# CityU-AIM-Group/SimT

Hardware: AMD Instinct MI355X
Metric: training images/sec at 768x768, DeepLabv2-R101+SimT (higher is better)
Workload: dtype bf16; 1 GPU; DeepLabv2-ResNet101 + SimT(C=19,K=3) full training iteration, batch=4/GPU, 768x768, bf16, 1xMI355X; global_batch=4, inputs=resident in HBM (see h2d_inclusive of a --full run for the PCIe-inclusive rate)

## Files before the change

### simt_amd/csrc/head_expand.hip

```cpp
#include "common.h"

struct TapArgs {
  const void* src;
  const float* bias;
  void* dst;
  int B, H, W, Q, QP, lds, ldd, ntaps;
  long M;
  short dy[SIMT_MAX_TAPS], dx[SIMT_MAX_TAPS];
};

__global__ __launch_bounds__(256) void tap_gather_sum_kernel(TapArgs a) {
  const int nq = a.QP >> 2;
  const long total = a.M * nq;
  const float* P = (const float*)a.src;
  float* y = (float*)a.dst;
  for (long idx = (long)blockIdx.x * blockDim.x + threadIdx.x; idx < total; idx += (long)gridDim.x * blockDim.x) {
    const int q = (int)(idx % nq);
    const long m = idx / nq;
    const int ox = (int)(m % a.W);
    const long t2 = m / a.W;
    const int oy = (int)(t2 % a.H);
    float4 acc = make_float4(0.f, 0.f, 0.f, 0.f);
    if (a.bias) {
      const int c = q * 4;
      acc.x = c + 0 < a.Q ? a.bias[c + 0] : 0.f;
      acc.y = c + 1 < a.Q ? a.bias[c + 1] : 0.f;
      acc.z = c + 2 < a.Q ? a.bias[c + 2] : 0.f;
      acc.w = c + 3 < a.Q ? a.bias[c + 3] : 0.f;
    }
    for (int t = 0; t < a.ntaps; ++t) {
      const int iy = oy + a.dy[t], ix = ox + a.dx[t];
      if (iy < 0 || iy >= a.H || ix < 0 || ix >= a.W) continue;
      const float4 v = *(const float4*)(P + (m + (long)a.dy[t] * a.W + a.dx[t]) * a.lds + t * a.QP + q * 4);
      acc.x += v.x; acc.y += v.y; acc.z += v.z; acc.w += v.w;
    }
    *(float4*)(y + m * a.ldd + q * 4) = acc;
  }
}

__global__ __launch_bounds__(256) void tap_scatter_kernel(TapArgs a) {
  const int ng = a.QP >> 3;
  const long total = a.M * a.ntaps * ng;
  const bf16_t* d = (const bf16_t*)a.src;
  bf16_t* G = (bf16_t*)a.dst;
  for (long idx = (long)blockIdx.x * blockDim.x + threadIdx.x; idx < total; idx += (long)gridDim.x * blockDim.x) {
    const int g = (int)(idx % ng);
    long r = idx / ng;
    const int t = (int)(r % a.ntaps);
    const long m = r / a.ntaps;
    const int ox = (int)(m % a.W);
    const int oy = (int)((m / a.W) % a.H);
    const int iy = oy - a.dy[t], ix = ox - a.dx[t];
    uint4 v = make_uint4(0u, 0u, 0u, 0u);
    if (iy >= 0 && iy < a.H && ix >= 0 && ix < a.W)
      v = *(const uint4*)(d + (m - ((long)a.dy[t] * a.W + a.dx[t])) * a.lds + g * 8);
    st_out16(G + m * a.ldd + t * a.QP + g * 8, v);
  }
}

static int tap_grid(long total) {
  long g = (total + 255) / 256;
  if (g > 256 * 16) g = 256 * 16;
  return (int)(g < 1 ? 1 : g);
}

extern "C" int simt_tap_gather_sum(const simt_tap_desc* d, simt_stream_t stream) {
  SIMT_CHECK(d && d->src && d->dst && d->ntaps >= 1 && d->ntaps <= SIMT_MAX_TAPS);
  SIMT_CHECK(d->QP % 4 == 0 && d->lds % 4 == 0 && d->ldd % 4 == 0 && d->QP <= d->ldd && d->ntaps * d->QP <= d->lds);
  TapArgs a;
  a.src = d->src; a.bias = d->bias; a.dst = d->dst; a.B = d->B; a.H = d->H; a.W = d->W; a.Q = d->Q; a.QP = d->QP;
  a.lds = d->lds; a.ldd = d->ldd; a.ntaps = d->ntaps; a.M = (long)d->B * d->H * d->W;
  for (int i = 0; i < SIMT_MAX_TAPS; ++i) { a.dy[i] = d->dy[i]; a.dx[i] = d->dx[i]; }
  hipLaunchKernelGGL(tap_gather_sum_kernel, dim3(tap_grid(a.M * (a.QP / 4))), dim3(256), 0, (hipStream_t)stream, a);
  SIMT_LAUNCH_CHECK();
  return SIMT_OK;
}

extern "C" int simt_tap_scatter(const simt_tap_desc* d, simt_stream_t stream) {
  SIMT_CHECK(d && d->src && d->dst && d->ntaps >= 1 && d->ntaps <= SIMT_MAX_TAPS);
  SIMT_CHECK(d->QP % 8 == 0 && d->lds % 8 == 0 && d->ldd % 8 == 0 && d->QP <= d->lds && d->ntaps * d->QP <= d->ldd);
  TapArgs a;
  a.src = d->src; a.bias = nullptr; a.dst = d->dst; a.B = d->B; a.H = d->H; a.W = d->W; a.Q = d->Q; a.QP = d->QP;
  a.lds = d->lds; a.ldd = d->ldd; a.ntaps = d->ntaps; a.M = (long)d->B * d->H * d->W;
  for (int i = 0; i < SIMT_MAX_TAPS; ++i) { a.dy[i] = d->dy[i]; a.dx[i] = d->dx[i]; }
  hipLaunchKernelGGL(tap_scatter_kernel, dim3(tap_grid(a.M * a.ntaps * (a.QP / 8))), dim3(256), 0, (hipStream_t)stream, a);
  SIMT_LAUNCH_CHECK();
  return SIMT_OK;
}
```

Before: 175.0 images/s.

## Add unrolled tap gather and row-batched tap scatter kernels with fast divmod

```diff
diff --git a/simt_amd/csrc/head_expand.hip b/simt_amd/csrc/head_expand.hip
--- a/simt_amd/csrc/head_expand.hip
+++ b/simt_amd/csrc/head_expand.hip
@@ -1,3 +1,4 @@
+#define SIMT_NT_STORES 1
 #include "common.h"
 
 struct TapArgs {
@@ -38,6 +39,40 @@
   }
 }
 
+template <int NT>
+__global__ __launch_bounds__(256) void tap_gather_sum_nt_kernel(TapArgs a, int nq, int total, float rcp_nq, float rcp_w, float rcp_h) {
+  const int idx = xcd_remap((int)blockIdx.x, (int)gridDim.x) * 256 + (int)threadIdx.x;
+  if (idx >= total) return;
+  int m, q, t2, ox, b, oy;
+  fast_divmod(idx, nq, rcp_nq, m, q);
+  fast_divmod(m, a.W, rcp_w, t2, ox);
+  fast_divmod(t2, a.H, rcp_h, b, oy);
+  const float* P = (const float*)a.src;
+  const float* own = P + (long)m * a.lds + q * 4;
+  const float* dummy = P + q * 4;
+  float4 v[NT];
+  bool in[NT];
+#pragma unroll
+  for (int t = 0; t < NT; ++t) {
+    const int iy = oy + a.dy[t], ix = ox + a.dx[t];
+    in[t] = iy >= 0 && iy < a.H && ix >= 0 && ix < a.W;
+    const long off = ((long)a.dy[t] * a.W + a.dx[t]) * a.lds + t * a.QP;
+    v[t] = *(const float4*)(in[t] ? own + off : dummy);
+  }
+  float4 acc = make_float4(0.f, 0.f, 0.f, 0.f);
+  if (a.bias) {
+    const int c = q * 4;
+    acc.x = c + 0 < a.Q ? a.bias[c + 0] : 0.f;
+    acc.y = c + 1 < a.Q ? a.bias[c + 1] : 0.f;
+    acc.z = c + 2 < a.Q ? a.bias[c + 2] : 0.f;
+    acc.w = c + 3 < a.Q ? a.bias[c + 3] : 0.f;
+  }
+#pragma unroll
+  for (int t = 0; t < NT; ++t)
+    if (in[t]) { acc.x += v[t].x; acc.y += v[t].y; acc.z += v[t].z; acc.w += v[t].w; }
+  *(float4*)((float*)a.dst + (long)m * a.ldd + q * 4) = acc;
+}
+
 __global__ __launch_bounds__(256) void tap_scatter_kernel(TapArgs a) {
   const int ng = a.QP >> 3;
   const long total = a.M * a.ntaps * ng;
@@ -58,6 +93,39 @@
   }
 }
 
+#ifndef TAP_ROWS
+#define TAP_ROWS 4
+#endif
+__global__ __launch_bounds__(256) void tap_scatter_rows_kernel(TapArgs a, int ng, int np, float rcp_ng, float rcp_w, float rcp_h) {
+  const int lane = (int)threadIdx.x & 63;
+  const int m0 = (xcd_remap((int)blockIdx.x, (int)gridDim.x) * 4 + ((int)threadIdx.x >> 6)) * TAP_ROWS;
+  const int M = (int)a.M;
+  if (m0 >= M) return;
+  int t2, ox0, b, oy0;
+  fast_divmod(m0, a.W, rcp_w, t2, ox0);
+  fast_divmod(t2, a.H, rcp_h, b, oy0);
+  const bf16_t* d = (const bf16_t*)a.src;
+  bf16_t* G = (bf16_t*)a.dst;
+  for (int j = lane; j < np; j += 64) {
+    int t, g;
+    fast_divmod(j, ng, rcp_ng, t, g);
+    const int dyt = a.dy[t], dxt = a.dx[t];
+    const long so = ((long)m0 - ((long)dyt * a.W + dxt)) * a.lds + g * 8;
+    uint4 v[TAP_ROWS];
+    int ox = ox0, oy = oy0;
+#pragma unroll
+    for (int r = 0; r < TAP_ROWS; ++r) {
+      const int iy = oy - dyt, ix = ox - dxt;
+      v[r] = make_uint4(0u, 0u, 0u, 0u);
+      if (m0 + r < M && iy >= 0 && iy < a.H && ix >= 0 && ix < a.W) v[r] = *(const uint4*)(d + so + (long)r * a.lds);
+      if (++ox == a.W) { ox = 0; if (++oy == a.H) oy = 0; }
+    }
+#pragma unroll
+    for (int r = 0; r < TAP_ROWS; ++r)
+      if (m0 + r < M) st_out16(G + (long)(m0 + r) * a.ldd + j * 8, v[r]);
+  }
+}
+
 static int tap_grid(long total) {
   long g = (total + 255) / 256;
   if (g > 256 * 16) g = 256 * 16;
@@ -71,7 +139,16 @@
   a.src = d->src; a.bias = d->bias; a.dst = d->dst; a.B = d->B; a.H = d->H; a.W = d->W; a.Q = d->Q; a.QP = d->QP;
   a.lds = d->lds; a.ldd = d->ldd; a.ntaps = d->ntaps; a.M = (long)d->B * d->H * d->W;
   for (int i = 0; i < SIMT_MAX_TAPS; ++i) { a.dy[i] = d->dy[i]; a.dx[i] = d->dx[i]; }
-  hipLaunchKernelGGL(tap_gather_sum_kernel, dim3(tap_grid(a.M * (a.QP / 4))), dim3(256), 0, (hipStream_t)stream, a);
+  const int nq = a.QP / 4;
+  const long total = a.M * nq;
+  if ((a.ntaps == 18 || a.ntaps == 36) && total < (1l << 24)) {
+    const dim3 grid((unsigned)((total + 255) / 256));
+    const float rq = 1.0f / (float)nq, rw = 1.0f / (float)a.W, rh = 1.0f / (float)a.H;
+    if (a.ntaps == 18) hipLaunchKernelGGL(tap_gather_sum_nt_kernel<18>, grid, dim3(256), 0, (hipStream_t)stream, a, nq, (int)total, rq, rw, rh);
+    else hipLaunchKernelGGL(tap_gather_sum_nt_kernel<36>, grid, dim3(256), 0, (hipStream_t)stream, a, nq, (int)total, rq, rw, rh);
+  } else {
+    hipLaunchKernelGGL(tap_gather_sum_kernel, dim3(tap_grid(total)), dim3(256), 0, (hipStream_t)stream, a);
+  }
   SIMT_LAUNCH_CHECK();
   return SIMT_OK;
 }
@@ -83,7 +160,14 @@
   a.src = d->src; a.bias = nullptr; a.dst = d->dst; a.B = d->B; a.H = d->H; a.W = d->W; a.Q = d->Q; a.QP = d->QP;
   a.lds = d->lds; a.ldd = d->ldd; a.ntaps = d->ntaps; a.M = (long)d->B * d->H * d->W;
   for (int i = 0; i < SIMT_MAX_TAPS; ++i) { a.dy[i] = d->dy[i]; a.dx[i] = d->dx[i]; }
-  hipLaunchKernelGGL(tap_scatter_kernel, dim3(tap_grid(a.M * a.ntaps * (a.QP / 8))), dim3(256), 0, (hipStream_t)stream, a);
+  const int ng = a.QP / 8, np = a.ntaps * ng;
+  if (a.M < (1l << 24)) {
+    const long waves = (a.M + TAP_ROWS - 1) / TAP_ROWS;
+    hipLaunchKernelGGL(tap_scatter_rows_kernel, dim3((unsigned)((waves + 3) / 4)), dim3(256), 0, (hipStream_t)stream, a, ng, np,
+                       1.0f / (float)ng, 1.0f / (float)a.W, 1.0f / (float)a.H);
+  } else {
+    hipLaunchKernelGGL(tap_scatter_kernel, dim3(tap_grid(a.M * np)), dim3(256), 0, (hipStream_t)stream, a);
+  }
   SIMT_LAUNCH_CHECK();
   return SIMT_OK;
 }
```

Result: no change. 174.8 images/s (-0.1%).
